# tmdt-buw/VQ-VAE-Transformer-Arc-Welding

Measured on AMD Instinct MI355X. Metric: welding windows/sec (train) VQ-VAE+8-blk Transformer at 1/2/4/8 MI355X, higher is better.
Workload: dtype bf16; 1 GPU; VQ-VAE-Patch reconstruction train step (configs[1]); global_batch=1024, per_gpu_batch=1024, seq_len=200, codebook=512x64, hidden=512, n_resblocks=8, patch=25, parallelism=dp1, optimizer=RAdam(lr 1e-3), operands=bf16 (opt-in), fp32 accumulation and master weights

## Files before the change

include/arcweld_amd.h:

```cpp
#ifndef ARCWELD_AMD_H
#define ARCWELD_AMD_H

#include <stdint.h>

#ifdef __cplusplus
extern "C" {
#endif

enum { AW_OK = 0, AW_ERR_ARG = -1, AW_ERR_LAUNCH = -2 };
enum { AW_F32 = 0, AW_BF16 = 1 };
enum { AW_ACT_GELU_ERF = 0, AW_ACT_GELU_TANH = 1, AW_ACT_DERIV = 2 };

const char* aw_last_error(void);
int aw_version(void);

typedef struct {
  int M, N, K;
  int a_dtype;
  const void* A; int64_t lda; int a_trans;
  const void* B; int64_t ldb; int b_trans;
  int conv_cin, conv_seg, conv_dir, conv_operand;
  float alpha, beta;
  const float* bias;
  int act;
  const float* pre; int64_t ld_pre;
  const float* resid; int64_t ld_resid;
  float drop_p; uint64_t drop_seed;
  void* C; int64_t ldc; int c_dtype;
  void* C2; int64_t ldc2; int c2_mode; int c2_dtype;
  float drop2_p; uint64_t drop2_seed;
  double* colstats; int stats_mod;
  float* a_rowsum;
  int bias_mod;
  int accumulate, col_mod, col_mul, col_off;
  const uint64_t* seed_ptr;
  int pre_dtype;
  int store_policy;
  int resid_dtype;
} aw_gemm_args;
#define AW_STORE_NT 0
#define AW_STORE_WT 1

int aw_gemm(const aw_gemm_args* args, void* stream);
int64_t aw_gemm_workspace(const aw_gemm_args* args);
int aw_gemm_ws(const aw_gemm_args* args, float* ws, int64_t ws_elems, void* stream);
#define AW_GEMM_MAX_GROUPS 16
int aw_gemm_grouped(const aw_gemm_args* args, int n, void* stream);
int aw_gemm_set_tile(int bm);
int aw_gemm_describe(const aw_gemm_args* args, int* layout, uint32_t* epi, int* tile_rows, int* specialised,
                     int* ragged, int* splits);
int aw_gemm_set_wgrad_policy(int mode);
#define AW_WGRAD_BATCH_MAX 32
int64_t aw_wgrad_batch_workspace(const aw_gemm_args* args, int n);
int aw_wgrad_batch(const aw_gemm_args* args, int n, void* ws, int64_t ws_bytes, void* stream);
int aw_wgrad_set_spin_limit(int polls);

#define AW_RES_CHAIN_MAX 16
typedef struct {
  int64_t N;
  int H, R;
  int taps, seg;
  const void* a0;
  const void* x0;
  const void* w1[AW_RES_CHAIN_MAX];
  const void* w2[AW_RES_CHAIN_MAX];
  const float* b1[AW_RES_CHAIN_MAX];
  const float* b2[AW_RES_CHAIN_MAX];
  void* dgelu_h[AW_RES_CHAIN_MAX];
  void* a1[AW_RES_CHAIN_MAX];
  void* dgelu_x[AW_RES_CHAIN_MAX];
  void* a[AW_RES_CHAIN_MAX];
  float drop_p;
  uint64_t drop_seed[AW_RES_CHAIN_MAX];
  const uint64_t* seed_ptr;
  int store_policy;
  uint64_t* drop_masks;
} aw_res_chain_fwd_args;
typedef struct {
  int64_t N;
  int H, R;
  int taps, seg;
  const void* gx;
  const void* gxo;
  const void* x0;
// ... 178 lines not shown
```

vq-vae-transformer-arc-welding_amd/arcweld/_native.py:

```python
from __future__ import annotations

import ctypes
import os

import torch

PKG_DIR = os.path.dirname(os.path.dirname(os.path.abspath(__file__)))
LIB_PATH = os.environ.get("ARCWELD_LIB") or os.path.join(PKG_DIR, "lib", "libarcweld_amd.so")
HEADER = os.path.join(os.path.dirname(PKG_DIR), "include", "arcweld_amd.h")

AW_F32, AW_BF16 = 0, 1
AW_ACT_GELU_ERF, AW_ACT_GELU_TANH, AW_ACT_DERIV = 0, 1, 2
AW_STORE_NT, AW_STORE_WT = 0, 1

c_i64 = ctypes.c_int64
c_int = ctypes.c_int
c_f = ctypes.c_float
c_p = ctypes.c_void_p


class GemmArgs(ctypes.Structure):
    _fields_ = [
        ("M", c_int), ("N", c_int), ("K", c_int),
        ("a_dtype", c_int),
        ("A", c_p), ("lda", c_i64), ("a_trans", c_int),
        ("B", c_p), ("ldb", c_i64), ("b_trans", c_int),
        ("conv_cin", c_int), ("conv_seg", c_int), ("conv_dir", c_int), ("conv_operand", c_int),
        ("alpha", c_f), ("beta", c_f),
        ("bias", c_p),
        ("act", c_int),
        ("pre", c_p), ("ld_pre", c_i64),
        ("resid", c_p), ("ld_resid", c_i64),
        ("drop_p", c_f), ("drop_seed", ctypes.c_uint64),
        ("C", c_p), ("ldc", c_i64), ("c_dtype", c_int),
        ("C2", c_p), ("ldc2", c_i64), ("c2_mode", c_int), ("c2_dtype", c_int),
        ("drop2_p", c_f), ("drop2_seed", ctypes.c_uint64),
        ("colstats", c_p), ("stats_mod", c_int),
        ("a_rowsum", c_p),
        ("bias_mod", c_int),
        ("accumulate", c_int), ("col_mod", c_int), ("col_mul", c_int), ("col_off", c_int),
        ("seed_ptr", c_p),
        ("pre_dtype", c_int),
        ("store_policy", c_int),
        ("resid_dtype", c_int),
    ]

# ... 9 lines not shown


OPS_PER_SEG = 2

RES_CHAIN_MAX = 16
RES_PACK_MAX = 32
_E = RES_CHAIN_MAX


class ResChainFwdArgs(ctypes.Structure):
    _fields_ = [("N", c_i64), ("H", c_int), ("R", c_int), ("taps", c_int), ("seg", c_int), ("a0", c_p), ("x0", c_p),
                ("w1", c_p * _E), ("w2", c_p * _E), ("b1", c_p * _E), ("b2", c_p * _E),
                ("dgelu_h", c_p * _E), ("a1", c_p * _E), ("dgelu_x", c_p * _E), ("a", c_p * _E),
                ("drop_p", c_f), ("drop_seed", ctypes.c_uint64 * _E), ("seed_ptr", c_p), ("store_policy", c_int),
                ("drop_masks", c_p)]


class ResChainBwdArgs(ctypes.Structure):
    _fields_ = [("N", c_i64), ("H", c_int), ("R", c_int), ("taps", c_int), ("seg", c_int), ("gx", c_p), ("gxo", c_p),
                ("x0", c_p), ("w1t", c_p * _E), ("w2t", c_p * _E), ("dgelu_h", c_p * _E), ("dgelu_x", c_p * _E),
                ("gh", c_p * _E), ("gxo_out", c_p * _E),
                ("drop_p", c_f), ("store_policy", c_int), ("drop_masks", c_p)]

SIGNATURES = {
    "aw_version": [],
    "aw_gemm": [ctypes.POINTER(GemmArgs), c_p],
    "aw_gemm_ws": [ctypes.POINTER(GemmArgs), c_p, c_i64, c_p],
    "aw_gemm_workspace": [ctypes.POINTER(GemmArgs)],
    "aw_gemm_grouped": [ctypes.POINTER(GemmArgs), c_int, c_p],
    "aw_gemm_set_tile": [c_int],
    "aw_gemm_describe": [ctypes.POINTER(GemmArgs), ctypes.POINTER(c_int), ctypes.POINTER(ctypes.c_uint32),
                         ctypes.POINTER(c_int), ctypes.POINTER(c_int), ctypes.POINTER(c_int), ctypes.POINTER(c_int)],
    "aw_gemm_set_wgrad_policy": [c_int],
    "aw_wgrad_batch_workspace": [ctypes.POINTER(GemmArgs), c_int],
    "aw_wgrad_batch": [ctypes.POINTER(GemmArgs), c_int, c_p, c_i64, c_p],
    "aw_wgrad_set_spin_limit": [c_int],
    "aw_res_chain_fwd": [ctypes.POINTER(ResChainFwdArgs), c_p],
    "aw_res_chain_bwd": [ctypes.POINTER(ResChainBwdArgs), c_p],
    "aw_res_pack_weights": [ctypes.POINTER(c_p), ctypes.POINTER(c_p), ctypes.POINTER(c_p), c_int, c_int, c_p],
    "aw_res_dropout_masks_bytes": [c_i64, c_int],
    "aw_res_dropout_masks": [c_i64, c_int, c_f, ctypes.POINTER(ctypes.c_uint64), c_p, c_p, c_p],
    "aw_weight_relayout_batch": [ctypes.POINTER(RelayoutJob), c_int, c_int, c_p],
    "aw_vq_forward": [c_p, c_p, c_i64, c_int, c_int, c_p, c_p, c_p, c_p, c_p],
    "aw_vq_forward_ex": [c_p, c_p, c_i64, c_int, c_int, c_p, c_p, c_p, c_p, c_p, c_int, c_p],
    "aw_vq_finalize": [c_p, c_p, c_i64, c_int, c_int, c_f, c_p, c_p, c_p],
    "aw_vq_forward_ex2": [c_p, c_p, c_i64, c_int, c_int, c_p, c_p, c_p, c_int, c_p, c_p, c_int, c_p],
    "aw_vq_finalize_ex": [c_p, c_int, c_p, c_i64, c_int, c_int, c_f, c_p, c_p, c_p],
    "aw_vq_backward": [c_p, c_p, c_p, c_p, c_p, c_i64, c_int, c_int, c_f, c_p, c_p, c_p],
    "aw_vq_backward_ex": [c_p, c_p, c_p, c_p, c_p, c_i64, c_int, c_int, c_f, c_p, c_p, c_p, c_int, c_p],
    "aw_vq_onehot": [c_p, c_i64, c_int, c_p, c_p],
    "aw_vq_gather": [c_p, c_p, c_i64, c_int, c_p, c_p],
    "aw_patchify": [c_p, c_i64, c_int, c_int, c_int, c_p, c_i64, c_int, c_p],
    "aw_weight_relayout": [c_p, c_int, c_int, c_int, c_int, c_int, c_p, c_i64, c_int, c_p],
    "aw_weight_grad_scatter": [c_p, c_int, c_int, c_int, c_int, c_int, c_i64, c_p, c_p],
    "aw_cast": [c_p, c_i64, c_p, c_int, c_p],
    "aw_unpatch_head_fwd": [c_p, c_i64, c_int, c_int, c_p, c_p, c_p, c_p, c_p],
    "aw_bn_finalize": [c_p, c_i64, c_int, c_p, c_p, c_p, c_p, c_p, c_f, c_f, c_int, c_p, c_p],
    "aw_unpatch_head_bwd1": [c_p, c_i64, c_int, c_int, c_p, c_p, c_p, c_p, c_p, c_p, c_p, c_p, c_p],
    "aw_unpatch_head_bwd2": [c_p, c_i64, c_int, c_int, c_p, c_p, c_p, c_p, c_int, c_p, c_int, c_p, c_p],
    "aw_unpatch_head_fwd_ex": [c_p, c_int, c_i64, c_int, c_int, c_p, c_p, c_p, c_p, c_p],
    "aw_unpatch_head_bwd1_ex": [c_p, c_int, c_i64, c_int, c_int, c_p, c_p, c_p, c_p, c_p, c_p, c_p, c_p, c_p],
    "aw_unpatch_head_fwd_bwd1": [c_p, c_int, c_i64, c_int, c_int, c_p, c_p, c_p, c_p, c_p, c_p, c_p, c_p, c_p, c_p,
                                 c_p, c_p, c_p, c_p],
    "aw_unpatch_head_bwd2_ex": [c_p, c_int, c_i64, c_int, c_int, c_p, c_p, c_p, c_p, c_int, c_p, c_int, c_p, c_p],
    "aw_bn_group_stats": [c_p, c_i64, c_int, c_int, c_p, c_p],
    "aw_bn_group_finalize": [c_p, c_i64, c_int, c_int, c_p, c_p, c_p, c_p, c_p, c_f, c_f, c_int, c_p, c_p],
# ... 104 lines not shown
```

vq-vae-transformer-arc-welding_amd/arcweld/kernels.py:

```python
from __future__ import annotations

import contextvars
import ctypes

import torch

from . import _native as nat
from ._native import AW_ACT_DERIV, AW_ACT_GELU_ERF, AW_ACT_GELU_TANH, AW_BF16, AW_F32, GemmArgs, call, dtype_code, ptr, stream_ptr

__all__ = ["gemm", "AW_ACT_DERIV", "AW_ACT_GELU_ERF", "AW_ACT_GELU_TANH", "AW_BF16", "AW_F32"]


def _ld(t):
    if t is None:
        return 0
    if t.dim() == 1:
        return t.shape[0]
    if t.stride(-1) != 1:
        raise nat.NativeError("operand rows must be contiguous (stride(-1) == 1)")
    return t.stride(0)


_STORE_POLICY = contextvars.ContextVar("arcweld_store_policy", default=0)

# ... 70 lines not shown
        if colstats.dtype != torch.float64:
            raise nat.NativeError("colstats must be float64")
        a.colstats, a.stats_mod = ptr(colstats), int(stats_mod)
    a.a_rowsum = ptr(a_rowsum)
    a.bias_mod = int(bias_mod)
    a.accumulate = int(bool(accumulate))
    a.col_mod, a.col_mul, a.col_off = (int(v) for v in col_map)
    a.seed_ptr = ptr(seed_ptr)
    return a


def _timed(s, fn, flops, tag, name=None, nbytes=None):
    e0, e1 = torch.cuda.Event(enable_timing=True), torch.cuda.Event(enable_timing=True)
    e0.record(s)
    fn(s.cuda_stream)
    e1.record(s)
    PROFILE.append((e0, e1, flops, tag, name or tag, nbytes))


def _gemm_tag(A):
    return "gemm_bf16" if A.dtype == torch.bfloat16 else "gemm_f32"


def gemm(A, B, M, N, K, *, stream=None, flops=None, **kw):
    a = _gemm_args(A, B, M, N, K, **kw)
    lib = nat.load()
    wsn = lib.aw_gemm_workspace(ctypes.byref(a))
    ws = torch.empty(wsn, device=A.device, dtype=torch.float32) if wsn > 0 else None
    if PROFILE is None:
        call("aw_gemm_ws", ctypes.byref(a), ptr(ws), wsn, stream_ptr(stream))
        return kw.get("C")
    s = stream if stream is not None else torch.cuda.current_stream()
    _timed(s, lambda sp: call("aw_gemm_ws", ctypes.byref(a), ptr(ws), wsn, sp),
           _algorithmic_flops(M, N, K, kw.get("conv"), flops), _gemm_tag(A), "gemm_kernel")
    return kw.get("C")


MAX_GROUPS = 16


def gemm_grouped(problems, stream=None):
    for c0 in range(0, len(problems), MAX_GROUPS):
        chunk = problems[c0:c0 + MAX_GROUPS]
        arr = (GemmArgs * len(chunk))(*[_gemm_args(A, B, M, N, K, **kw) for (A, B, M, N, K, kw) in chunk])
        if PROFILE is None:
            call("aw_gemm_grouped", arr, len(chunk), stream_ptr(stream))
            continue
        s = stream if stream is not None else torch.cuda.current_stream()
        fl = sum(_algorithmic_flops(M, N, K, kw.get("conv"), None) for (_, _, M, N, K, kw) in chunk)
        c0_ = chunk[0]
        nm = "wgrad_conv3_kernel" if (c0_[5].get("conv") is not None and c0_[0].dtype == torch.bfloat16) \
            else "gemm_kernel (grouped)"
        _timed(s, lambda sp: call("aw_gemm_grouped", arr, len(chunk), sp), fl, _gemm_tag(chunk[0][0]), nm)


WGRAD_BATCH_MAX = 32


def wgrad_batch_ok(problems):
    import os
    mode = os.environ.get("ARCWELD_WGRAD_BATCH", "auto")
    if mode == "0" or not problems or len(problems) > WGRAD_BATCH_MAX:
        return False
    arr = (GemmArgs * len(problems))(*[_gemm_args(A, B, M, N, K, **kw) for (A, B, M, N, K, kw) in problems])
    if nat.load().aw_wgrad_batch_workspace(arr, len(problems)) <= 0:
        return False
    tiles = sum((M // 256) * (N // 256) for (_, _, M, N, _, _) in problems)
    return mode == "1" or tiles >= 128


def wgrad_batch(problems, stream=None):
    arr = (GemmArgs * len(problems))(*[_gemm_args(A, B, M, N, K, **kw) for (A, B, M, N, K, kw) in problems])
    lib = nat.load()
    wsb = lib.aw_wgrad_batch_workspace(arr, len(problems))
    if wsb < 0:
        raise nat.NativeError(f"aw_wgrad_batch: batch not eligible ({lib.aw_last_error().decode(errors='replace')})")
    ws = torch.empty((wsb + 3) // 4, device=problems[0][0].device, dtype=torch.float32)
    if PROFILE is None:
        call("aw_wgrad_batch", arr, len(problems), ptr(ws), wsb, stream_ptr(stream))
        return
    s = stream if stream is not None else torch.cuda.current_stream()
    fl = sum(_algorithmic_flops(M, N, K, None, None) for (_, _, M, N, K, _) in problems)
    _timed(s, lambda sp: call("aw_wgrad_batch", arr, len(problems), ptr(ws), wsb, sp), fl, _gemm_tag(problems[0][0]),
           "wgrad_tt_kernel")

# ... 546 lines not shown
```

vq-vae-transformer-arc-welding_amd/csrc/gemm.hip:

```cpp
#include <stdlib.h>

#include "gemm_core.h"

using namespace awg;

namespace {

template <typename T, Layout LY>
void launch_generic(const GemmP& P, hipStream_t s, bool ragged) {
  if (ragged) launch_kernel<T, LY, true, EP_GENERIC, 128>(P, s);
  else launch_tiled<T, LY, EP_GENERIC>(P, s);
}

Layout layout_of(const aw_gemm_args& a) {
  const bool conv = a.conv_cin > 0;
  const bool aconv = conv && a.conv_operand == 0, bconv = conv && a.conv_operand == 1;
  if (!a.a_trans && !a.b_trans) return aconv ? L_NN_CONV : L_NN;
  if (!a.a_trans && a.b_trans) return aconv ? L_NT_CONV : L_NT;
  if (a.a_trans && !a.b_trans) return L_TN;
  return bconv ? L_TT_KCONV : L_TT;
}

uint32_t epi_code(const aw_gemm_args& a, const GemmP& P, bool ragged) {
  if (P.splits > 1 || a.accumulate) return ragged ? EP_GENERIC : EP_ACCUM;
// ... 232 lines not shown
  if (a.a_dtype == AW_BF16 && !is_ragged(a) && (g_tile_override == 256 || (g_tile_override == 0 && auto256))) {
    bm = 256;
    if (a.accumulate && t256 < 240 && a.K >= 24 * BK) {
      splits = 256 / t256;
      if (splits > a.K / (12 * BK)) splits = a.K / (12 * BK);
      if (grouped && splits > AW_GROUPED_MAXSPLIT) splits = AW_GROUPED_MAXSPLIT;
      if (splits < 1) splits = 1;
    }
  }
  if (bm == 128) {
    const int nb = aw_cdiv(a.M, 128) * P.tiles_n * ngroups;
    if (plain && nb < 384 && a.K >= 24 * BK) {
      splits = 512 / nb;
      const int max_splits = a.K / ((nb <= 16 ? min_ksteps_small() : AW_SPLIT_MIN_KSTEPS) * BK);
      if (splits > max_splits) splits = max_splits;
      if (grouped && splits > AW_GROUPED_MAXSPLIT) splits = AW_GROUPED_MAXSPLIT;
      if (splits < 1) splits = 1;
    }
    if (grouped && a.accumulate && nb > 512 && nb < 1024 && a.K >= 48 * BK) {
      splits = 2;
    }
  }
  P.bm = bm;
  P.tiles_per_group = aw_cdiv(a.M, bm) * P.tiles_n;
  P.nblocks = P.tiles_per_group * ngroups;
  P.ksplit = splits > 1 ? aw_cdiv(aw_cdiv(a.K, splits), BK) * BK : (a.K > 0 ? a.K : 1);
  P.splits = splits > 1 ? aw_cdiv(a.K, P.ksplit) : 1;
}

static bool wants_slabs(const aw_gemm_args& a, const GemmP& P) { return P.splits > 1 && P.bm == 128 && (a.beta == 0.f || a.beta == 1.f || a.accumulate); }

extern "C" int64_t aw_gemm_workspace(const aw_gemm_args* a) {
  if (!a || a->M <= 0 || a->N <= 0) return 0;
  GemmP P;
  plan(*a, 1, false, P);
  return wants_slabs(*a, P) ? (int64_t)P.splits * a->M * a->N : 0;
}

extern "C" int aw_gemm_ws(const aw_gemm_args* args, float* ws, int64_t ws_elems, void* stream) {
  if (!args) {
    aw::set_error("aw_gemm: null args");
    return AW_ERR_ARG;
  }
  const aw_gemm_args& a = *args;
  if (int st = validate(a)) return st;
  if (a.M == 0 || a.N == 0) return AW_OK;
  GemmP P;
  plan(a, 1, false, P);
  if (wants_slabs(a, P) && ws && ws_elems >= (int64_t)P.splits * a.M * a.N) P.ws = ws;
  hipStream_t s = reinterpret_cast<hipStream_t>(stream);
  if (P.splits > 1 && !P.ws && a.beta == 0.f && !a.accumulate) {
    if (hipMemset2DAsync(a.C, a.ldc * sizeof(float), 0, a.N * sizeof(float), a.M, s) != hipSuccess)
      return aw::check_launch("aw_gemm split-K zero");
  }
  const bool ragged = is_ragged(a);
  if (a.a_dtype == AW_BF16)
    dispatch<bf16>(P, s, ragged);
  else
    dispatch<float>(P, s, ragged);
  if (P.ws) {
    const int64_t n = (int64_t)a.M * a.N;
    int64_t g = ((a.N & 3) == 0 ? n / 4 + 255 : n + 255) / 256;
    if (g > 2048) g = 2048;
    hipLaunchKernelGGL(gemm_reduce_kernel, dim3((int)g), dim3(256), 0, s, P.ws, P.splits, a.M, a.N, a);
  }
  return aw::check_launch("aw_gemm");
}

extern "C" int aw_gemm_describe(const aw_gemm_args* args, int* layout, uint32_t* epi, int* tile_rows,
                                int* specialised, int* ragged, int* splits) {
  if (!args) {
    aw::set_error("aw_gemm_describe: null args");
    return AW_ERR_ARG;
  }
  const aw_gemm_args& a = *args;
  if (int st = validate(a)) return st;
  const bool rg = is_ragged(a);
  const Layout ly = layout_of(a);
  uint32_t code = EP_GENERIC;
  int bm = 0, nsplit = 0;
  bool fast = false;
  if (a.M > 0 && a.N > 0) {
    GemmP P;
    plan(a, 1, false, P);
    code = epi_code(a, P, rg);
    fast = fast_kernel(P, nullptr, a.a_dtype == AW_BF16, ly, code, false);
    bm = P.bm;
    nsplit = P.splits;
  }
  if (layout) *layout = (int)ly;
  if (epi) *epi = code;
  if (tile_rows) *tile_rows = bm;
  if (specialised) *specialised = fast ? 1 : 0;
  if (ragged) *ragged = rg ? 1 : 0;
  if (splits) *splits = nsplit;
  return AW_OK;
}

extern "C" int aw_gemm_grouped(const aw_gemm_args* args, int n, void* stream) {
  AW_REQUIRE(args && n >= 1 && n <= AW_GEMM_MAX_GROUPS, "aw_gemm_grouped: need 1..%d problems", AW_GEMM_MAX_GROUPS);
  const aw_gemm_args& a = args[0];
  for (int g = 0; g < n; ++g) {
    if (int st = validate(args[g])) return st;
    const aw_gemm_args& b = args[g];
    const bool same = b.M == a.M && b.N == a.N && b.K == a.K && b.a_dtype == a.a_dtype && b.lda == a.lda &&
                      b.a_trans == a.a_trans && b.ldb == a.ldb && b.b_trans == a.b_trans &&
                      b.conv_cin == a.conv_cin && b.conv_seg == a.conv_seg && b.conv_dir == a.conv_dir &&
                      b.conv_operand == a.conv_operand && b.alpha == a.alpha && b.beta == a.beta &&
                      b.ldc == a.ldc && b.c_dtype == a.c_dtype && b.accumulate == a.accumulate &&
                      b.col_mod == a.col_mod && b.col_mul == a.col_mul && b.col_off == a.col_off &&
                      (b.a_rowsum == nullptr) == (a.a_rowsum == nullptr) && b.C != nullptr;
    AW_REQUIRE(same, "aw_gemm_grouped: problem %d differs from problem 0 in more than A, B, C, a_rowsum", g);
  }
  AW_REQUIRE(a.accumulate && !a.C2 && !a.bias && !a.colstats, "aw_gemm_grouped: accumulate-mode problems only");
  if (a.M == 0 || a.N == 0) return AW_OK;
  if (wgrad_conv3_try(args, n, reinterpret_cast<hipStream_t>(stream))) return aw::check_launch("aw_gemm_grouped");
  GemmP P;
  plan(a, n, true, P);
  for (int g = 0; g < n; ++g) {
    P.gA[g] = args[g].A;
    P.gB[g] = args[g].B;
    P.gC[g] = args[g].C;
    P.gRow[g] = args[g].a_rowsum;
  }
  hipStream_t s = reinterpret_cast<hipStream_t>(stream);
  const bool ragged = is_ragged(a);
  if (a.a_dtype == AW_BF16)
    dispatch<bf16>(P, s, ragged);
  else
    dispatch<float>(P, s, ragged);
  return aw::check_launch("aw_gemm_grouped");
}
```

vq-vae-transformer-arc-welding_amd/csrc/gemm_core.h:

```cpp
#pragma once
#include "common.h"

#pragma clang diagnostic ignored "-Winline-asm"

namespace awg {

constexpr int BN = 128;
constexpr int ROWB = 128;
constexpr int CPITCH = BN + 4;

template <int BMT> struct Cfg;
#ifndef AW_W8
#define AW_W8 1
#endif
#if AW_W8
template <> struct Cfg<128> { static constexpr int NTH = 512, NSTAGE = 2, MINB = 4; };
#else
template <> struct Cfg<128> { static constexpr int NTH = 256, NSTAGE = 2, MINB = 2; };
#endif
template <> struct Cfg<256> { static constexpr int NTH = 512, NSTAGE = 3, MINB = 1; };
template <int BMT> constexpr int stage_bytes() { return (BMT + BN) * ROWB; }
template <int BMT> constexpr int smem_bytes() {
  return Cfg<BMT>::NSTAGE * stage_bytes<BMT>() > BMT * CPITCH * 4 ? Cfg<BMT>::NSTAGE * stage_bytes<BMT>()
                                                                   : BMT * CPITCH * 4;
// ... 766 lines not shown

enum Layout { L_NN = 0, L_NN_CONV = 1, L_NT = 2, L_NT_CONV = 3, L_TN = 4, L_TT = 5, L_TT_KCONV = 6 };

template <Layout LY> struct LayoutArgs;
template <> struct LayoutArgs<L_NN> { static constexpr bool ATR = false, BTR = false; static constexpr int AC = CONV_NONE, BC = CONV_NONE; };
template <> struct LayoutArgs<L_NN_CONV> { static constexpr bool ATR = false, BTR = false; static constexpr int AC = CONV_ROWSHIFT, BC = CONV_NONE; };
template <> struct LayoutArgs<L_NT> { static constexpr bool ATR = false, BTR = true; static constexpr int AC = CONV_NONE, BC = CONV_NONE; };
template <> struct LayoutArgs<L_NT_CONV> { static constexpr bool ATR = false, BTR = true; static constexpr int AC = CONV_ROWSHIFT, BC = CONV_NONE; };
template <> struct LayoutArgs<L_TN> { static constexpr bool ATR = true, BTR = false; static constexpr int AC = CONV_NONE, BC = CONV_NONE; };
template <> struct LayoutArgs<L_TT> { static constexpr bool ATR = true, BTR = true; static constexpr int AC = CONV_NONE, BC = CONV_NONE; };
template <> struct LayoutArgs<L_TT_KCONV> { static constexpr bool ATR = true, BTR = true; static constexpr int AC = CONV_NONE, BC = CONV_KSHIFT; };

template <typename T, Layout LY, bool RAGGED, uint32_t EPI, int BMT>
inline void launch_kernel(const GemmP& P, hipStream_t s) {
  using LA = LayoutArgs<LY>;
  hipLaunchKernelGGL((gemm_kernel<T, LA::ATR, LA::BTR, LA::AC, LA::BC, RAGGED, EPI, BMT>), dim3(P.nblocks, P.splits),
                     dim3(Cfg<BMT>::NTH), 0, s, P);
}

template <typename T, Layout LY, uint32_t EPI>
inline void launch_tiled(const GemmP& P, hipStream_t s) {
  if constexpr (sizeof(T) == 2 && (EPI == EP_GENERIC || EPI == EP_ACCUM)) {
    if (P.bm == 256) {
      launch_kernel<T, LY, false, EPI, 256>(P, s);
      return;
    }
  }
  launch_kernel<T, LY, false, EPI, 128>(P, s);
}

bool launch_fast_fwd(const GemmP& P, hipStream_t s, bool is_bf16, Layout ly, uint32_t code, bool launch);
bool launch_fast_bwd(const GemmP& P, hipStream_t s, bool is_bf16, Layout ly, uint32_t code, bool launch);
bool launch_fast_256(const GemmP& P, hipStream_t s, Layout ly, uint32_t code, bool launch);
bool wgrad_conv3_try(const aw_gemm_args* args, int n, hipStream_t s);


}
```

vq-vae-transformer-arc-welding_amd/csrc/wgrad.hip:

```cpp
#include "gemm_core.h"

#include <stdlib.h>

#include <algorithm>

#pragma clang diagnostic ignored "-Winline-asm"

namespace {

constexpr int W3_BM = 256;
constexpr int W3_CB = 64;
constexpr int W3_BK = 64;
constexpr int W3_NTH = 512;
constexpr int W3_A = W3_BK * W3_BM * 2;
constexpr int W3_B = W3_BK * W3_CB * 2;
constexpr int W3_BUF = W3_A + W3_B;
constexpr int W3_NBUF = 4;
constexpr int W3_DMA = 5;

struct W3Params {
  int M, cin, K, seg, ngroups, tiles_m, tiles_i, nblocks;
  int lda, ldb, ldc;
  int col_mod, col_mul, col_off;
  float alpha;
// ... 190 lines not shown
    __builtin_amdgcn_s_setprio(0);
    w3_barrier();
  }
  if (wr == 0) w3_barrier();

  const float alpha = P.alpha;
  float* C = P.C[grp];
#pragma unroll
  for (int f = 0; f < 3; ++f) {
    const int c = wc * 48 + 16 * f + li;
    const int n = (c >> 6) * P.cin + ci0 + (c & 63);
    const int64_t oc = P.col_mod > 0 ? (int64_t)(n % P.col_mod) * P.col_mul + n / P.col_mod + P.col_off
                                     : (int64_t)n * (P.col_mul > 0 ? P.col_mul : 1) + P.col_off;
#pragma unroll
    for (int i = 0; i < 8; ++i) {
      const int row = m0 + wr * 128 + 16 * i + 4 * g;
      float* d = C + (int64_t)row * P.ldc + oc;
      float v[4];
#pragma unroll
      for (int r = 0; r < 4; ++r) v[r] = d[(int64_t)r * P.ldc];
#pragma unroll
      for (int r = 0; r < 4; ++r) d[(int64_t)r * P.ldc] = v[r] + alpha * acc[i][f][r];
    }
  }
  if (tile_rowsum && li == 0) {
#pragma unroll
    for (int j = 0; j < 2; ++j)
#pragma unroll
      for (int r = 0; r < 4; ++r) atomicAdd(rowptr + m0 + wr * 128 + 16 * (2 * wcu + j) + 4 * g + r, alpha * rs[j][r]);
  }
}

int g_policy = 0;

constexpr int WT_BM = 256, WT_BN = 256, WT_BK = 32, WT_NTH = 512;
constexpr int WT_A = WT_BK * WT_BM * 2;
constexpr int WT_B = WT_BK * WT_BN * 2;
constexpr int WT_BUF = WT_A + WT_B;
constexpr int WT_NBUF = 4;
constexpr int WT_DMA = 4;
constexpr int WT_SLAB = WT_BM * WT_BN;
constexpr int WT_MAXTILES = 8192;

struct WTProb {
  const void* A;
  const void* B;
  float* C;
  float* rowsum;
  int64_t lda, ldb, ldc;
  int M, N, tiles_n, tile0;
  int col_mod, col_mul, col_off;
};

struct WTParams {
  WTProb p[AW_WGRAD_BATCH_MAX];
  int nprob, K, nk, G, total_tiles, S, units;
  int big;
  float alpha;
  float* ws;
  int spin;
};

__device__ int g_wt_arrive[WT_MAXTILES];
__device__ int g_wt_pub[WT_MAXTILES];

__device__ __forceinline__ v4i32 wt_desc(const void* base, int64_t nbytes) {
// ... 302 lines not shown
    q.col_mul = a.col_mul;
    q.col_off = a.col_off;
    t0 += (a.M / WT_BM) * q.tiles_n;
  }
  P->nprob = n;
  P->K = a0.K;
  P->nk = (a0.K + WT_BK - 1) / WT_BK;
  P->total_tiles = tiles;
  const int cus = wt_cus();
  int best = 1;
  int64_t best_cost = INT64_MAX;
  for (int S = 1; S <= 4; S *= 2) {
    if (S > 1 && P->nk / S < 16) break;
    const int64_t units = (int64_t)tiles * S, rounds = (units + cus - 1) / cus;
    const int64_t cost = rounds * ((P->nk + S - 1) / S);
    if (cost < best_cost) {
      best_cost = cost;
      best = S;
    }
  }
  P->S = best;
  static const bool mixed = [] { const char* e = getenv("AW_WGRAD_MIXED"); return !(e && atoi(e) == 0); }();
  P->big = (mixed && best == 2 && tiles > cus && 2 * (tiles - cus) <= cus) ? cus : 0;
  P->units = P->big + (tiles - P->big) * best;
  P->G = std::min(cus, P->units);
  P->alpha = a0.alpha;
  return AW_OK;
}

}

namespace awg {

bool wgrad_conv3_try(const aw_gemm_args* args, int n, hipStream_t s) {
  const aw_gemm_args& a = args[0];
  if (g_policy < 0) return false;
  const int cin = a.conv_cin;
  const bool shape = a.a_dtype == AW_BF16 && a.a_trans && a.b_trans && cin > 0 && a.conv_operand == 1 &&
                     a.N == 3 * cin && a.M % W3_BM == 0 && cin % W3_CB == 0 && a.K % W3_BK == 0 && a.K > 0 &&
                     (a.conv_seg == 8 || a.conv_seg == 16 || a.conv_seg == 32) && a.accumulate && a.beta == 0.f &&
                     a.c_dtype == AW_F32 && a.lda % 8 == 0 && a.ldb % 8 == 0;
  if (!shape) return false;
  const int tiles = (a.M / W3_BM) * (cin / W3_CB);
  if (g_policy == 0 && tiles * n < 128) return false;
  const int64_t ea = ((int64_t)a.K - 1) * a.lda + a.M, eb = ((int64_t)a.K - 1) * a.ldb + cin;
  if (ea * 2 >= 0x7FFFFFF0 || eb * 2 >= 0x7FFFFFF0) return false;
  W3Params P;
  memset(&P, 0, sizeof(P));
  P.M = a.M;
  P.cin = cin;
  P.K = a.K;
  P.seg = a.conv_seg;
  P.ngroups = n;
  P.tiles_m = a.M / W3_BM;
  P.tiles_i = cin / W3_CB;
  P.nblocks = tiles * n;
  P.lda = (int)a.lda;
  P.ldb = (int)a.ldb;
  P.ldc = (int)a.ldc;
  P.col_mod = a.col_mod;
  P.col_mul = a.col_mul;
  P.col_off = a.col_off;
  P.alpha = a.alpha;
  for (int g = 0; g < n; ++g) {
    P.A[g] = args[g].A;
    P.B[g] = args[g].B;
    P.C[g] = reinterpret_cast<float*>(args[g].C);
    P.rowsum[g] = args[g].a_rowsum;
  }
  hipLaunchKernelGGL(wgrad_conv3_kernel, dim3(P.nblocks), dim3(W3_NTH), 0, s, P);
  return true;
}

}

extern "C" int aw_gemm_set_wgrad_policy(int mode) {
  AW_REQUIRE(mode >= -1 && mode <= 1, "aw_gemm_set_wgrad_policy: mode must be -1, 0 or 1");
  g_policy = mode;
  return AW_OK;
}


extern "C" int64_t aw_wgrad_batch_workspace(const aw_gemm_args* args, int n) {
  WTParams P;
  if (wt_plan(args, n, &P) != AW_OK) return -1;
  return P.S > 1 ? (int64_t)P.units * WT_SLAB * (int64_t)sizeof(float) : 16;
}

extern "C" int aw_wgrad_batch(const aw_gemm_args* args, int n, void* ws, int64_t ws_bytes, void* stream) {
  WTParams P;
  if (int st = wt_plan(args, n, &P)) return st;
  AW_REQUIRE(ws && ((uintptr_t)ws % 16) == 0 &&
                 ws_bytes >= (P.S > 1 ? (int64_t)P.units * WT_SLAB * (int64_t)sizeof(float) : 16),
             "aw_wgrad_batch: workspace must be 16-B aligned and hold aw_wgrad_batch_workspace() bytes");
  P.ws = reinterpret_cast<float*>(ws);
  P.spin = g_wt_spin;
  hipLaunchKernelGGL(wgrad_tt_kernel, dim3(P.G), dim3(WT_NTH), 0, reinterpret_cast<hipStream_t>(stream), P);
  return aw::check_launch("aw_wgrad_batch");
}

extern "C" int aw_wgrad_set_spin_limit(int polls) {
  AW_REQUIRE(polls >= 0, "aw_wgrad_set_spin_limit: polls must be >= 0");
  g_wt_spin = polls;
  return AW_OK;
}

// ... 1 lines not shown
```

Before: 423,300 windows/s.

## Add specialised weight-gradient linear kernel with split-K slabs and DMA ring

Result: no change. 427,000 windows/s, median of 6 (+0.9%).

```diff
diff --git a/include/arcweld_amd.h b/include/arcweld_amd.h
--- a/include/arcweld_amd.h
+++ b/include/arcweld_amd.h
@@ -50,6 +50,10 @@
 int aw_gemm_describe(const aw_gemm_args* args, int* layout, uint32_t* epi, int* tile_rows, int* specialised,
                      int* ragged, int* splits);
 int aw_gemm_set_wgrad_policy(int mode);
+#define AW_WGRAD_KERNEL_GEMM 0
+#define AW_WGRAD_KERNEL_CONV3 1
+#define AW_WGRAD_KERNEL_LIN 2
+int aw_wgrad_describe(const aw_gemm_args* args, int n, int slabs, int* kernel, int* units, int* splits);
 #define AW_WGRAD_BATCH_MAX 32
 int64_t aw_wgrad_batch_workspace(const aw_gemm_args* args, int n);
 int aw_wgrad_batch(const aw_gemm_args* args, int n, void* ws, int64_t ws_bytes, void* stream);
diff --git a/vq-vae-transformer-arc-welding_amd/arcweld/_native.py b/vq-vae-transformer-arc-welding_amd/arcweld/_native.py
--- a/vq-vae-transformer-arc-welding_amd/arcweld/_native.py
+++ b/vq-vae-transformer-arc-welding_amd/arcweld/_native.py
@@ -12,6 +12,7 @@
 AW_F32, AW_BF16 = 0, 1
 AW_ACT_GELU_ERF, AW_ACT_GELU_TANH, AW_ACT_DERIV = 0, 1, 2
 AW_STORE_NT, AW_STORE_WT = 0, 1
+AW_WGRAD_KERNEL_GEMM, AW_WGRAD_KERNEL_CONV3, AW_WGRAD_KERNEL_LIN = 0, 1, 2
 
 c_i64 = ctypes.c_int64
 c_int = ctypes.c_int
@@ -87,6 +88,8 @@
     "aw_gemm_describe": [ctypes.POINTER(GemmArgs), ctypes.POINTER(c_int), ctypes.POINTER(ctypes.c_uint32),
                          ctypes.POINTER(c_int), ctypes.POINTER(c_int), ctypes.POINTER(c_int), ctypes.POINTER(c_int)],
     "aw_gemm_set_wgrad_policy": [c_int],
+    "aw_wgrad_describe": [ctypes.POINTER(GemmArgs), c_int, c_int, ctypes.POINTER(c_int), ctypes.POINTER(c_int),
+                          ctypes.POINTER(c_int)],
     "aw_wgrad_batch_workspace": [ctypes.POINTER(GemmArgs), c_int],
     "aw_wgrad_batch": [ctypes.POINTER(GemmArgs), c_int, c_p, c_i64, c_p],
     "aw_wgrad_set_spin_limit": [c_int],
diff --git a/vq-vae-transformer-arc-welding_amd/arcweld/kernels.py b/vq-vae-transformer-arc-welding_amd/arcweld/kernels.py
--- a/vq-vae-transformer-arc-welding_amd/arcweld/kernels.py
+++ b/vq-vae-transformer-arc-welding_amd/arcweld/kernels.py
@@ -126,11 +126,27 @@
         return kw.get("C")
     s = stream if stream is not None else torch.cuda.current_stream()
     _timed(s, lambda sp: call("aw_gemm_ws", ctypes.byref(a), ptr(ws), wsn, sp),
-           _algorithmic_flops(M, N, K, kw.get("conv"), flops), _gemm_tag(A), "gemm_kernel")
+           _algorithmic_flops(M, N, K, kw.get("conv"), flops), _gemm_tag(A),
+           wgrad_kernel_name(a, 1, slabs=True) if ws is not None else "gemm_kernel")
     return kw.get("C")
 
 
 MAX_GROUPS = 16
+
+_WGRAD_KERNELS = {nat.AW_WGRAD_KERNEL_GEMM: "gemm_kernel", nat.AW_WGRAD_KERNEL_CONV3: "wgrad_conv3_kernel",
+                  nat.AW_WGRAD_KERNEL_LIN: "wgrad_lin_kernel"}
+
+
+def wgrad_describe(arr, n, slabs=False):
+    kern, units, splits = ctypes.c_int(0), ctypes.c_int(0), ctypes.c_int(0)
+    call("aw_wgrad_describe", arr if n > 1 or not isinstance(arr, GemmArgs) else ctypes.byref(arr), n, int(slabs),
+         ctypes.byref(kern), ctypes.byref(units), ctypes.byref(splits))
+    return kern.value, units.value, splits.value
+
+
+def wgrad_kernel_name(arr, n, slabs=False):
+    name = _WGRAD_KERNELS[wgrad_describe(arr, n, slabs)[0]]
+    return name + " (grouped)" if name == "gemm_kernel" and not slabs else name
 
 
 def gemm_grouped(problems, stream=None):
@@ -142,9 +158,7 @@
             continue
         s = stream if stream is not None else torch.cuda.current_stream()
         fl = sum(_algorithmic_flops(M, N, K, kw.get("conv"), None) for (_, _, M, N, K, kw) in chunk)
-        c0_ = chunk[0]
-        nm = "wgrad_conv3_kernel" if (c0_[5].get("conv") is not None and c0_[0].dtype == torch.bfloat16) \
-            else "gemm_kernel (grouped)"
+        nm = wgrad_kernel_name(arr, len(chunk))
         _timed(s, lambda sp: call("aw_gemm_grouped", arr, len(chunk), sp), fl, _gemm_tag(chunk[0][0]), nm)
 
 
diff --git a/vq-vae-transformer-arc-welding_amd/csrc/gemm.hip b/vq-vae-transformer-arc-welding_amd/csrc/gemm.hip
--- a/vq-vae-transformer-arc-welding_amd/csrc/gemm.hip
+++ b/vq-vae-transformer-arc-welding_amd/csrc/gemm.hip
@@ -288,6 +288,7 @@
 
 extern "C" int64_t aw_gemm_workspace(const aw_gemm_args* a) {
   if (!a || a->M <= 0 || a->N <= 0) return 0;
+  if (int S = wgrad_lin_try(a, 1, true, nullptr, 0, nullptr, false, nullptr)) return (int64_t)S * a->M * a->N;
   GemmP P;
   plan(*a, 1, false, P);
   return wants_slabs(*a, P) ? (int64_t)P.splits * a->M * a->N : 0;
@@ -305,15 +306,22 @@
   plan(a, 1, false, P);
   if (wants_slabs(a, P) && ws && ws_elems >= (int64_t)P.splits * a.M * a.N) P.ws = ws;
   hipStream_t s = reinterpret_cast<hipStream_t>(stream);
+  const int lin = ws ? wgrad_lin_try(args, 1, true, ws, ws_elems, s, true, nullptr) : 0;
+  if (lin) {
+    P.ws = ws;
+    P.splits = lin;
+  }
   if (P.splits > 1 && !P.ws && a.beta == 0.f && !a.accumulate) {
     if (hipMemset2DAsync(a.C, a.ldc * sizeof(float), 0, a.N * sizeof(float), a.M, s) != hipSuccess)
       return aw::check_launch("aw_gemm split-K zero");
   }
   const bool ragged = is_ragged(a);
-  if (a.a_dtype == AW_BF16)
+  if (lin) {
+  } else if (a.a_dtype == AW_BF16) {
     dispatch<bf16>(P, s, ragged);
-  else
+  } else {
     dispatch<float>(P, s, ragged);
+  }
   if (P.ws) {
     const int64_t n = (int64_t)a.M * a.N;
     int64_t g = ((a.N & 3) == 0 ? n / 4 + 255 : n + 255) / 256;
@@ -353,7 +361,7 @@
   return AW_OK;
 }
 
-extern "C" int aw_gemm_grouped(const aw_gemm_args* args, int n, void* stream) {
+static int validate_grouped(const aw_gemm_args* args, int n) {
   AW_REQUIRE(args && n >= 1 && n <= AW_GEMM_MAX_GROUPS, "aw_gemm_grouped: need 1..%d problems", AW_GEMM_MAX_GROUPS);
   const aw_gemm_args& a = args[0];
   for (int g = 0; g < n; ++g) {
@@ -369,8 +377,16 @@
     AW_REQUIRE(same, "aw_gemm_grouped: problem %d differs from problem 0 in more than A, B, C, a_rowsum", g);
   }
   AW_REQUIRE(a.accumulate && !a.C2 && !a.bias && !a.colstats, "aw_gemm_grouped: accumulate-mode problems only");
+  return AW_OK;
+}
+
+extern "C" int aw_gemm_grouped(const aw_gemm_args* args, int n, void* stream) {
+  if (int st = validate_grouped(args, n)) return st;
+  const aw_gemm_args& a = args[0];
   if (a.M == 0 || a.N == 0) return AW_OK;
-  if (wgrad_conv3_try(args, n, reinterpret_cast<hipStream_t>(stream))) return aw::check_launch("aw_gemm_grouped");
+  hipStream_t s = reinterpret_cast<hipStream_t>(stream);
+  if (wgrad_conv3_try(args, n, s, true)) return aw::check_launch("aw_gemm_grouped");
+  if (wgrad_lin_try(args, n, false, nullptr, 0, s, true, nullptr)) return aw::check_launch("aw_gemm_grouped");
   GemmP P;
   plan(a, n, true, P);
   for (int g = 0; g < n; ++g) {
@@ -379,7 +395,6 @@
     P.gC[g] = args[g].C;
     P.gRow[g] = args[g].a_rowsum;
   }
-  hipStream_t s = reinterpret_cast<hipStream_t>(stream);
   const bool ragged = is_ragged(a);
   if (a.a_dtype == AW_BF16)
     dispatch<bf16>(P, s, ragged);
@@ -387,3 +402,33 @@
     dispatch<float>(P, s, ragged);
   return aw::check_launch("aw_gemm_grouped");
 }
+
+extern "C" int aw_wgrad_describe(const aw_gemm_args* args, int n, int slabs, int* kernel, int* units, int* splits) {
+  int kern = AW_WGRAD_KERNEL_GEMM, nu = 0, ns = 0;
+  if (slabs) {
+    AW_REQUIRE(args && n == 1, "aw_wgrad_describe: the slab form takes one problem");
+    if (int st = validate(args[0])) return st;
+  } else if (int st = validate_grouped(args, n)) {
+    return st;
+  }
+  const aw_gemm_args& a = args[0];
+  if (a.M > 0 && a.N > 0) {
+    if (!slabs && wgrad_conv3_try(args, n, nullptr, false)) {
+      kern = AW_WGRAD_KERNEL_CONV3;
+      nu = (a.M / 256) * (a.conv_cin / 64) * n;
+      ns = 1;
+    } else if (int S = wgrad_lin_try(args, n, slabs != 0, nullptr, 0, nullptr, false, &nu)) {
+      kern = AW_WGRAD_KERNEL_LIN;
+      ns = S;
+    } else {
+      GemmP P;
+      plan(a, n, !slabs, P);
+      nu = P.nblocks * P.splits;
+      ns = P.splits;
+    }
+  }
+  if (kernel) *kernel = kern;
+  if (units) *units = nu;
+  if (splits) *splits = ns;
+  return AW_OK;
+}
diff --git a/vq-vae-transformer-arc-welding_amd/csrc/gemm_core.h b/vq-vae-transformer-arc-welding_amd/csrc/gemm_core.h
--- a/vq-vae-transformer-arc-welding_amd/csrc/gemm_core.h
+++ b/vq-vae-transformer-arc-welding_amd/csrc/gemm_core.h
@@ -822,7 +822,9 @@
 bool launch_fast_fwd(const GemmP& P, hipStream_t s, bool is_bf16, Layout ly, uint32_t code, bool launch);
 bool launch_fast_bwd(const GemmP& P, hipStream_t s, bool is_bf16, Layout ly, uint32_t code, bool launch);
 bool launch_fast_256(const GemmP& P, hipStream_t s, Layout ly, uint32_t code, bool launch);
-bool wgrad_conv3_try(const aw_gemm_args* args, int n, hipStream_t s);
-
-
-}
+bool wgrad_conv3_try(const aw_gemm_args* args, int n, hipStream_t s, bool launch);
+int wgrad_lin_try(const aw_gemm_args* args, int n, bool slabs, float* ws, int64_t ws_elems, hipStream_t s, bool launch,
+                  int* units);
+
+
+}
diff --git a/vq-vae-transformer-arc-welding_amd/csrc/wgrad.hip b/vq-vae-transformer-arc-welding_amd/csrc/wgrad.hip
--- a/vq-vae-transformer-arc-welding_amd/csrc/wgrad.hip
+++ b/vq-vae-transformer-arc-welding_amd/csrc/wgrad.hip
@@ -246,6 +246,236 @@
 }
 
 int g_policy = 0;
+
+#ifndef AW_WL_BK
+#define AW_WL_BK 64
+#endif
+constexpr int WL_BM = 256, WL_BN = 128, WL_BK = AW_WL_BK, WL_NTH = 512;
+static_assert(WL_BK == 64 || WL_BK == 32, "K-tile of 64 or 32 tokens");
+constexpr int WL_KU = WL_BK / 32;
+constexpr int WL_A = WL_BK * WL_BM * 2;
+constexpr int WL_B = WL_BK * WL_BN * 2;
+constexpr int WL_BUF = WL_A + WL_B;
+constexpr int WL_NBUF = 192 / WL_BK;
+constexpr int WL_LA = WL_NBUF - 1;
+constexpr int WL_DA = WL_BK / 16, WL_DB = WL_BK / 32;
+constexpr int WL_DMA = WL_DA + WL_DB;
+constexpr int WL_TP = WL_BN + 4;
+static_assert(WL_BM * WL_TP * 4 <= WL_NBUF * WL_BUF, "the epilogue tile lives in the ring");
+
+struct WLParams {
+  int M, N, K, tiles_m, tiles_n, splits, nunits;
+  int lda, ldb, ldc;
+  int col_mod, col_mul, col_off;
+  float alpha;
+  float* ws;
+  const void* A[AW_GEMM_MAX_GROUPS];
+  const void* B[AW_GEMM_MAX_GROUPS];
+  float* C[AW_GEMM_MAX_GROUPS];
+  float* rowsum[AW_GEMM_MAX_GROUPS];
+};
+
+__device__ __forceinline__ v4i32 wl_desc(const char* base, int64_t nbytes) {
+  const uint64_t b = (uint64_t)(uintptr_t)base;
+  return v4i32{(int)__builtin_amdgcn_readfirstlane((uint32_t)b),
+               (int)__builtin_amdgcn_readfirstlane((uint32_t)(b >> 32) & 0xFFFFu),
+               (int)__builtin_amdgcn_readfirstlane((uint32_t)nbytes), 0x00020000};
+}
+
+__device__ __forceinline__ int wl_key(int k) { return (k & 3) | (((k >> 3) & 1) << 2); }
+
+__device__ __forceinline__ void wl_retire(int newer) {
+  static_assert(4 * WL_DMA < 64 && WL_LA <= 5, "vmcnt immediates");
+  if (newer <= 0) w3_vmcnt<0>();
+  else if (newer == 1) w3_vmcnt<WL_DMA>();
+  else if (newer == 2) w3_vmcnt<2 * WL_DMA>();
+  else if (newer == 3) w3_vmcnt<3 * WL_DMA>();
+  else w3_vmcnt<4 * WL_DMA>();
+}
+
+__global__ __launch_bounds__(WL_NTH, 1) void wgrad_lin_kernel(WLParams P) {
+  __shared__ __attribute__((aligned(16))) char smem[WL_NBUF * WL_BUF];
+  const int tid = threadIdx.x, lane = tid & 63, wid = tid >> 6;
+  const int wr = wid >> 2, wc = wid & 3;
+  const int g = lane >> 4, li = lane & 15, q = li >> 2, p = li & 3;
+
+  int unit = awg::xcd_remap(blockIdx.x, P.nunits);
+  const int per_group = P.tiles_m * P.tiles_n;
+  const int grp = unit / (per_group * P.splits);
+  unit -= grp * per_group * P.splits;
+  const int sp = unit / per_group;
+  unit -= sp * per_group;
+  const int tm = unit / P.tiles_n, tn = unit - tm * P.tiles_n;
+  const int m0 = tm * WL_BM, n0 = tn * WL_BN;
+  const int nkt = P.K / WL_BK;
+  const int k0 = (int)((int64_t)sp * nkt / P.splits), k1 = (int)((int64_t)(sp + 1) * nkt / P.splits);
+  const int nk = k1 - k0;
+  const int64_t a_step = (int64_t)WL_BK * P.lda * 2, b_step = (int64_t)WL_BK * P.ldb * 2;
+  const char* Ag = reinterpret_cast<const char*>(P.A[grp]) + (int64_t)m0 * 2 + k0 * a_step;
+  const char* Bg = reinterpret_cast<const char*>(P.B[grp]) + (int64_t)n0 * 2 + k0 * b_step;
+  const int64_t extA = (((int64_t)nk * WL_BK - 1) * P.lda + WL_BM) * 2;
+  const int64_t extB = (((int64_t)nk * WL_BK - 1) * P.ldb + WL_BN) * 2;
+
+  int offA[WL_DA], offB[WL_DB];
+#pragma unroll
+  for (int i = 0; i < WL_DA; ++i) {
+    const int c = tid + WL_NTH * i;
+    {
+      const int k = c >> 5, s = (c & 31) >> 1, half = c & 1;
+      offA[i] = (k * P.lda + ((s & 8) | ((s & 7) ^ wl_key(k))) * 16 + half * 8) * 2;
+    }
+    if (i < WL_DB) {
+      const int k = c >> 4, s = (c & 15) >> 1, half = c & 1;
+      offB[i] = (k * P.ldb + (s ^ wl_key(k)) * 16 + half * 8) * 2;
+    }
+  }
+  const uint32_t lds0 = (uint32_t)(uintptr_t)(__attribute__((address_space(3))) char*)smem;
+  const uint32_t wave_dst = (uint32_t)__builtin_amdgcn_readfirstlane((uint32_t)(tid & ~63)) * 16u;
+
+  auto dma = [&](int t, int slot) {
+    const uint32_t buf = lds0 + (uint32_t)(slot * WL_BUF);
+    const v4i32 da = wl_desc(Ag + t * a_step, extA - t * a_step);
+    const v4i32 db = wl_desc(Bg + t * b_step, extB - t * b_step);
+#pragma unroll
+    for (int i = 0; i < WL_DA; ++i) w3_dma(buf + wave_dst + (uint32_t)(i * WL_NTH * 16), offA[i], da);
+#pragma unroll
+    for (int i = 0; i < WL_DB; ++i) w3_dma(buf + WL_A + wave_dst + (uint32_t)(i * WL_NTH * 16), offB[i], db);
+  };
+
+  const int key = q | ((g & 1) << 2);
+  int fa[4], fb[4];
+#pragma unroll
+  for (int i = 0; i < 4; ++i) {
+    fa[i] = (8 * g + q) * (WL_BM * 2) + 256 * (wc >> 1) + 32 * ((((wc & 1) * 4 + i) ^ key)) + 8 * p;
+    fb[i] = WL_A + (8 * g + q) * (WL_BN * 2) + 32 * ((wr * 4 + i) ^ key) + 8 * p;
+  }
+
+  float* rowptr = P.rowsum[grp];
+  const bool unit_rowsum = rowptr != nullptr && wr == 0;
+  int rs_count = (tn - k0 % P.tiles_n + P.tiles_n) % P.tiles_n;
+  const uint4 ones = make_uint4(0x3F803F80u, 0x3F803F80u, 0x3F803F80u, 0x3F803F80u);
+  f32x4 rs[4];
+  f32x4 acc[4][4];
+#pragma unroll
+  for (int i = 0; i < 4; ++i) {
+    rs[i] = f32x4{0.f, 0.f, 0.f, 0.f};
+#pragma unroll
+    for (int f = 0; f < 4; ++f) acc[i][f] = f32x4{0.f, 0.f, 0.f, 0.f};
+  }
+
+  const int wru = __builtin_amdgcn_readfirstlane(wr);
+#pragma unroll
+  for (int j = 0; j < WL_LA; ++j)
+    if (j < nk) dma(j, j);
+  wl_retire(min(nk, WL_LA) - 1);
+  w3_barrier();
+  if (wru == 1) {
+    if (WL_LA < nk) dma(WL_LA, WL_LA);
+    w3_barrier();
+  }
+
+  uint4 af[WL_KU][4], bfr[WL_KU][4];
+  int slot = 0;
+  for (int t = 0; t < nk; ++t) {
+    const char* buf = smem + slot * WL_BUF;
+    {
+      constexpr int AK = WL_BM * 2, BKB = WL_BN * 2;
+#pragma unroll
+      for (int u = 0; u < WL_KU; ++u) {
+#pragma unroll
+        for (int i = 0; i < 4; ++i)
+          af[u][i] = w3_tr(buf + fa[i] + 32 * u * AK, buf + fa[i] + (32 * u + 4) * AK);
+#pragma unroll
+        for (int f = 0; f < 4; ++f)
+          bfr[u][f] = w3_tr(buf + fb[f] + 32 * u * BKB, buf + fb[f] + (32 * u + 4) * BKB);
+      }
+    }
+    const int newer = min(nk - 1, t + WL_LA) - (t + 1);
+    if (wru == 0) {
+      if (t + WL_LA < nk) dma(t + WL_LA, slot == 0 ? WL_NBUF - 1 : slot - 1);
+    } else {
+      wl_retire(newer);
+    }
+    asm volatile("s_waitcnt lgkmcnt(0)" ::: "memory");
+    w3_barrier();
+    if (wru == 1 && t + 1 + WL_LA < nk) dma(t + 1 + WL_LA, slot);
+    __builtin_amdgcn_s_setprio(1);
+#pragma unroll
+    for (int u = 0; u < WL_KU; ++u)
+#pragma unroll
+      for (int i = 0; i < 4; ++i)
+#pragma unroll
+        for (int f = 0; f < 4; ++f)
+          acc[i][f] = __builtin_amdgcn_mfma_f32_16x16x32_bf16(__builtin_bit_cast(bf16x8, af[u][i]),
+                                                             __builtin_bit_cast(bf16x8, bfr[u][f]), acc[i][f], 0, 0, 0);
+    const bool rs_now = unit_rowsum && rs_count == 0;
+    rs_count = rs_count == 0 ? P.tiles_n - 1 : rs_count - 1;
+    if (rs_now) {
+#pragma unroll
+      for (int u = 0; u < WL_KU; ++u)
+#pragma unroll
+        for (int i = 0; i < 4; ++i)
+          rs[i] = __builtin_amdgcn_mfma_f32_16x16x32_bf16(__builtin_bit_cast(bf16x8, af[u][i]),
+                                                         __builtin_bit_cast(bf16x8, ones), rs[i], 0, 0, 0);
+    }
+    __builtin_amdgcn_s_setprio(0);
+    if (wru == 0) wl_retire(newer);
+    w3_barrier();
+    slot = slot == WL_NBUF - 1 ? 0 : slot + 1;
+  }
+  if (wr == 0) w3_barrier();
+
+  const float alpha = P.alpha;
+  if (unit_rowsum && li == 0) {
+#pragma unroll
+    for (int i = 0; i < 4; ++i)
+#pragma unroll
+      for (int r = 0; r < 4; ++r) atomicAdd(rowptr + m0 + wc * 64 + 16 * i + 4 * g + r, alpha * rs[i][r]);
+  }
+  float* T = reinterpret_cast<float*>(smem);
+#pragma unroll
+  for (int i = 0; i < 4; ++i)
+#pragma unroll
+    for (int f = 0; f < 4; ++f)
+#pragma unroll
+      for (int r = 0; r < 4; ++r) T[(wc * 64 + 16 * i + 4 * g + r) * WL_TP + wr * 64 + 16 * f + li] = acc[i][f][r];
+  __syncthreads();
+  float* C = P.C[grp];
+  const bool vec = P.col_mod == 0 && P.col_mul <= 1 && (P.ldc & 3) == 0 && (P.col_off & 3) == 0 &&
+                   (((uintptr_t)C) & 15) == 0;
+  if (P.ws != nullptr || (P.splits == 1 && vec)) {
+    const int c4 = (tid & 31) * 4, rr = tid >> 5;
+    const bool slab = P.ws != nullptr;
+    float* D = slab ? P.ws + ((int64_t)sp * P.M + m0) * P.N + n0 + c4 : C + (int64_t)m0 * P.ldc + P.col_off + n0 + c4;
+    const int64_t ldd = slab ? P.N : P.ldc;
+#pragma unroll
+    for (int k0r = 0; k0r < 16; k0r += 8) {
+      f32x4 old[8];
+#pragma unroll
+      for (int k = 0; k < 8; ++k) {
+        const int row = rr + 16 * (k0r + k);
+        old[k] = slab ? f32x4{0.f, 0.f, 0.f, 0.f} : *reinterpret_cast<const f32x4*>(D + row * ldd);
+      }
+#pragma unroll
+      for (int k = 0; k < 8; ++k) {
+        const int row = rr + 16 * (k0r + k);
+        const f32x4 a = *reinterpret_cast<const f32x4*>(T + row * WL_TP + c4);
+        *reinterpret_cast<f32x4*>(D + row * ldd) = slab ? a : old[k] + alpha * a;
+      }
+    }
+  } else {
+    const int cc = tid & 127, rr = tid >> 7;
+    const int n = n0 + cc;
+    const int64_t oc = P.col_mod > 0 ? (int64_t)(n % P.col_mod) * P.col_mul + n / P.col_mod + P.col_off
+                                     : (int64_t)n * (P.col_mul > 0 ? P.col_mul : 1) + P.col_off;
+    float* D = C + (int64_t)m0 * P.ldc + oc;
+#pragma unroll 8
+    for (int k = 0; k < 64; ++k) {
+      const int row = rr + 4 * k;
+      atomicAdd(D + (int64_t)row * P.ldc, alpha * T[row * WL_TP + cc]);
+    }
+  }
+}
 
 constexpr int WT_BM = 256, WT_BN = 256, WT_BK = 32, WT_NTH = 512;
 constexpr int WT_A = WT_BK * WT_BM * 2;
@@ -614,7 +844,7 @@
 
 namespace awg {
 
-bool wgrad_conv3_try(const aw_gemm_args* args, int n, hipStream_t s) {
+bool wgrad_conv3_try(const aw_gemm_args* args, int n, hipStream_t s, bool launch) {
   const aw_gemm_args& a = args[0];
   if (g_policy < 0) return false;
   const int cin = a.conv_cin;
@@ -627,6 +857,7 @@
   if (g_policy == 0 && tiles * n < 128) return false;
   const int64_t ea = ((int64_t)a.K - 1) * a.lda + a.M, eb = ((int64_t)a.K - 1) * a.ldb + cin;
   if (ea * 2 >= 0x7FFFFFF0 || eb * 2 >= 0x7FFFFFF0) return false;
+  if (!launch) return true;
   W3Params P;
   memset(&P, 0, sizeof(P));
   P.M = a.M;
@@ -654,6 +885,58 @@
   return true;
 }
 
+int wgrad_lin_try(const aw_gemm_args* args, int n, bool slabs, float* ws, int64_t ws_elems, hipStream_t s, bool launch,
+                  int* units) {
+  const aw_gemm_args& a = args[0];
+  if (g_policy < 0) return 0;
+  const bool shape = a.a_dtype == AW_BF16 && a.a_trans && a.b_trans && a.conv_cin == 0 && a.M > 0 && a.N > 0 &&
+                     a.M % WL_BM == 0 && a.N % WL_BN == 0 && a.K >= 64 && a.K % 64 == 0 && a.accumulate &&
+                     a.beta == 0.f && a.c_dtype == AW_F32 && a.C && a.lda % 8 == 0 && a.ldb % 8 == 0 &&
+                     a.lda >= a.M && a.ldb >= a.N && a.ldc < 0x7FFFFFFF;
+  if (!shape) return 0;
+  const int64_t ea = ((int64_t)a.K - 1) * a.lda + a.M, eb = ((int64_t)a.K - 1) * a.ldb + a.N;
+  if (ea * 2 >= 0x7FFFFFF0 || eb * 2 >= 0x7FFFFFF0) return 0;
+  const int64_t tiles = (int64_t)(a.M / WL_BM) * (a.N / WL_BN) * n;
+  const int nkt = a.K / 64, cus = wt_cus();
+  if (tiles > 0x3FFFFFFF) return 0;
+  int S = 1;
+  if (slabs) {
+    S = (int)std::min<int64_t>(std::min<int64_t>(cus / tiles, 8), nkt / 8);
+    if (S < 2 || (int64_t)a.M * a.N * S >= 0x7FFFFFFF) return 0;
+  } else if (2 * tiles <= cus && nkt >= 2) {
+    S = 2;
+  }
+  if (g_policy == 0 && 2 * tiles * S < cus) return 0;
+  if (units) *units = (int)tiles * S;
+  if (!launch) return S;
+  if (slabs && (!ws || ((uintptr_t)ws % 16) != 0 || ws_elems < (int64_t)S * a.M * a.N)) return 0;
+  WLParams P;
+  memset(&P, 0, sizeof(P));
+  P.M = a.M;
+  P.N = a.N;
+  P.K = a.K;
+  P.tiles_m = a.M / WL_BM;
+  P.tiles_n = a.N / WL_BN;
+  P.splits = S;
+  P.nunits = (int)tiles * S;
+  P.lda = (int)a.lda;
+  P.ldb = (int)a.ldb;
+  P.ldc = (int)a.ldc;
+  P.col_mod = a.col_mod;
+  P.col_mul = a.col_mul;
+  P.col_off = a.col_off;
+  P.alpha = a.alpha;
+  P.ws = slabs ? ws : nullptr;
+  for (int g = 0; g < n; ++g) {
+    P.A[g] = args[g].A;
+    P.B[g] = args[g].B;
+    P.C[g] = reinterpret_cast<float*>(args[g].C);
+    P.rowsum[g] = args[g].a_rowsum;
+  }
+  hipLaunchKernelGGL(wgrad_lin_kernel, dim3(P.nunits), dim3(WL_NTH), 0, s, P);
+  return S;
+}
+
 }
 
 extern "C" int aw_gemm_set_wgrad_policy(int mode) {
```
